# alexaiken/mpas-regent

Measured on AMD Instinct MI355X. Metric: Mcell-columns/sec per RK3 step; achieved HBM GB/s; x1.163842×56L, higher is better.
Workload: dtype f64; 1 GPU; x1.163842 x 56 levels, atm_srk3 (3 dyn_tend rk 0/1/2, 7 acoustic substeps); nCells=163842, nEdges=491520, nVertices=327680, nVertLevels=56, parallelism=single-gpu, exact=0, physics=0, transport=0, graph=1, fusedamp=1, fusesetup=1, smlsum=1, fusesml=1, defer4=1, ntu=1, mdamp=0

## Files before the change

mpas-regent_amd/csrc/k_acoustic.hip:

```cpp
#include "k_cols.h"
#include "mpas_dev.h"
#include "mpas_halo.h"

#include <type_traits>

namespace mpas {

template <int LP>
__device__ __forceinline__ double damp_edge(double rup, double d1, double d2, double t12, double spec, double coef,
                                            bool on) {
    return on ? rup + coef * (d2 - d1) * (1.0 - spec) / t12 : rup;
}

template <int LP, bool TME>
__device__ __forceinline__ void acoustic_orph_body(const DevState& S, double coefp, int ob) {
    const int L = S.L, k = (int)(threadIdx.x % LP);
    const int j = col_of<LP>(ob);
    if (j >= S.n_orph) return;
    const int e = fi(S, X_orph)[j];
    const int c1 = fi(S, F_cellsOnEdge)[(size_t)e * 2], c2 = fi(S, F_cellsOnEdge)[(size_t)e * 2 + 1];
    const double *dvi = fd(S, X_dvB), *tmf = fd(S, F_theta_m);
    const double ru = colk(fd(S, F_ru_p), e), d1 = colk(dvi, c1), d2 = colk(dvi, c2);
    const double t12 = TME ? colk(fd(S, X_tme), e) : colk(tmf, c1) + colk(tmf, c2);
    const int sh1 = fi(S, F_isShared)[c1], sh2 = fi(S, F_isShared)[c2];
    const bool on = (k < L) & !(sh1 & sh2);
    colk(fw(S, X_rupB), e) = PADW(damp_edge<LP>(ru, d1, d2, t12, fd(S, F_specZoneMaskEdge)[e], coefp, on));
}
template <int LP, bool TME>
__global__ __launch_bounds__(256) void k_acoustic_orph(DevState S, double coefp) {
    acoustic_orph_body<LP, TME>(S, coefp, (int)blockIdx.x);
}

template <int LP, bool EXACT, bool SELF, bool FIRST, bool MPASV, int MODE, bool TME, int SML, bool ACO = false,
          bool DD0 = false>
__device__ __forceinline__ void acoustic_body(const DevState& S, double dts, int small_step, double epssm, double resm,
                                              double coefp, int ncb, Blk bk, int wold = 1, int ddx = 0,
                                              double dtseps = 0.0) {
    static_assert(!(MPASV && MODE), "the deferred damping is the reference semantics' (physics 0)");
    static_assert(!(MPASV && ACO), "the MPAS forms load the stored set (recover changes theta_m)");
    static_assert(!(MPASV && DD0), "the MPAS forms' recover writes rw");
    static_assert(!(TME && ACO), "option tmedge keeps the stored set (its exact first launch would lose a wave)");
    static_assert(!SML || (FIRST && !MPASV), "set_smlstep precedes a stage's first substep (reference semantics)");
    static_assert(SML != 2 || !EXACT, "the flux sum reassociates: fast path only");
    const int L = S.L, k = (int)(threadIdx.x % LP);
    int blk = bk.b;
    blk = xcd_block_n(S.xcd, blk, ncb);
    const int c = col_of<LP>(blk) + S.lo[KC];
    if (c >= S.nCO) return;
    const size_t p = (size_t)c * LP + lpos(LP, k);
    double* rtp_f = fw(S, F_rtheta_pp);
    double* rpp_f = fw(S, F_rho_pp);
    double* rwp_f = fw(S, F_rw_p);
    double* ww_f = fw(S, F_wwAvg);
    const bool kl = k < L;
    const double spec = fd(S, F_specZoneMaskCell)[c];
    const int* eoc = fi(S, F_edgesOnCell) + (size_t)c * 10;
    const double* sgn = fd(S, F_edgesOnCellSign) + (size_t)c * 10;
    const int *cc1 = fi(S, X_ce_c1) + (size_t)c * 10, *cc2 = fi(S, X_ce_c2) + (size_t)c * 10;
    const double* cdv = fd(S, X_ce_dv) + (size_t)c * 10;
    const double invA = fd(S, F_invAreaCell)[c];
    const double *ru_p = fd(S, F_ru_p), *tm_f = fd(S, F_theta_m);
    const int *coth = fi(S, X_ce_oth) + (size_t)c * 10, *cs1 = fi(S, X_ce_s1) + (size_t)c * 10;
    int e_[NF], c1_[NF], c2_[NF], o_[NF], s1_[NF];
    double sgn_[NF], cdv_[NF], rup_[NF], t1_[NF], t2_[NF], ts_[NF];
    const int ne = SELF ? cell_rec<true>(S, c, e_, o_, s1_) : cell_rec<false>(S, c, e_, c1_, c2_);
    row_ld(sgn, sgn_);
    row_ld(cdv, cdv_);
    double rtp, rpp, rwp, ww, tm, tend_rho, w, coftz, zz, rz, cofwt, cofwz, cofwr, a_tri, alpha, rws, rw, dss;
    if constexpr (FIRST) {
        rtp = rpp = rwp = ww = 0.0;
    } else {
        col_rd2<LP>(rtp_f, rpp_f, c, k, L, rtp, rpp);
        col_rd2<LP>(rwp_f, ww_f, c, k, L, rwp, ww);
    }
    col_rd2<LP>(fd(S, F_theta_m), fd(S, F_tend_rho), c, k, L, tm, tend_rho);
    const uint8_t cpr = SML ? ((const uint8_t*)S.f[F_cprMask])[p] : 0;
    static_assert(NF % 2 == 0, "slot pairs");
#pragma unroll
    for (int i = 0; i < NF; i += 2) {
        gather2s<LP>(ru_p, e_[i], e_[i + 1], k, rup_[i], rup_[i + 1]);
        if constexpr (TME) {
            gather2s<LP>(fd(S, X_tme), e_[i], e_[i + 1], k, ts_[i], ts_[i + 1]);
        } else {
            cell_pair2<LP, SELF>(tm_f, c1_, c2_, o_, s1_, tm, i, k, t1_[i], t2_[i], t1_[i + 1], t2_[i + 1]);
            ts_[i] = t2_[i] + t1_[i];
            ts_[i + 1] = t2_[i + 1] + t1_[i + 1];
        }
    }
    int own = 0;
    if constexpr (MODE == 2) {
        const double* dvi = fd(S, X_dvB);
        const int* sh = fi(S, F_isShared);
        const double* spz = fd(S, F_specZoneMaskEdge);
        own = fi(S, X_eown)[c];
        const double dv_c = SELF ? colk(dvi, c) : 0.0;
        double d1_[NF], d2_[NF];
#pragma unroll
        for (int i = 0; i < NF; i += 2)
            cell_pair2<LP, SELF>(dvi, c1_, c2_, o_, s1_, dv_c, i, k, d1_[i], d2_[i], d1_[i + 1], d2_[i + 1]);
        int sh1_[NF], sh2_[NF];
        double spz_[NF];
#pragma unroll
        for (int i = 0; i < NF; i++) {
            const int x1 = SELF ? (s1_[i] ? c : o_[i]) : c1_[i], x2 = SELF ? (s1_[i] ? o_[i] : c) : c2_[i];
            sh1_[i] = sh[x1];
            sh2_[i] = sh[x2];
            spz_[i] = LP == 64 ? uniform_d(spz[e_[i]]) : spz[e_[i]];
        }
#pragma unroll
        for (int i = 0; i < NF; i++) {
            const bool on = kl & (e_[i] < S.nEdges) & !(sh1_[i] & sh2_[i]);
            rup_[i] = damp_edge<LP>(rup_[i], d1_[i], d2_[i], ts_[i], spz_[i], coefp, on);
        }
    }
    if constexpr (!ACO) col_rd2<LP>(fd(S, F_w), fd(S, F_coftz), c, k, L, w, coftz);
    else if constexpr (DD0) w = col_rd<LP>(fd(S, F_w), c, k, L);
    else if (ddx) col_rd2<LP>(fd(S, F_w), fd(S, F_dss), c, k, L, w, dss);
    else col_rd2<LP>(fd(S, F_w), fd(S, F_rw), c, k, L, w, rw);
    col_rd2<LP>(fd(S, F_zz), fd(S, F_rho_zz), c, k, L, zz, rz);
    const double fzm = fd(S, F_fzm)[k], fzp = fd(S, F_fzp)[k];
    int wst = 0;
    if constexpr (SML == 2) {
        double wn = w - colk(fd(S, X_smlS), c);
        wn *= (fzm * zz + fzp * lvl_dn<LP>(zz, k));
        const bool rz_ok = fi(S, F_bdyMaskCell)[c] <= kRelaxZone;
        wst = ((k <= L) & rz_ok & (cpr != 0)) ? 1 : ((k > L) & rz_ok) ? 2 : 0;
        if (wst == 1) w = wn;
    } else if constexpr (SML == 1) {
        const double* ut_f = fd(S, F_u_tend);
        const double *zb = fd(S, F_zb_cell), *zb3 = fd(S, F_zb3_cell);
        const double* sgnc = fd(S, F_edgesOnCell_sign) + (size_t)c * 10;
        double ut_[NF], utm_[NF], zb_[NF], zb3_[NF], sgs_[NF];
        row_ld(sgnc, sgs_);
#pragma unroll
        for (int i = 0; i < NF; i += 2) gather2s<LP>(ut_f, e_[i], e_[i + 1], k, ut_[i], ut_[i + 1]);
#pragma unroll
        for (int i = 0; i < NF; i++) {
            ut_[i] = ldz(k <= L, ut_[i]);
            gather2<LP>(zb, c * 10 + i, zb3, c * 10 + i, k, zb_[i], zb3_[i]);
        }
#pragma unroll
        for (int i = 0; i < NF; i++) utm_[i] = lvl_dn<LP>(ut_[i], k);
        double wn = w, sum = 0.0;
#pragma unroll
        for (int i = 0; i < NF; i++) {
            double flux = sgs_[i] * (fzm * ut_[i] + fzp * utm_[i]);
            const double t = (zb_[i] + copysign(1.0, ut_[i]) * zb3_[i]) * flux;
            if constexpr (EXACT) wn = sub_if(i < ne, wn, t);
            else sum = add_if(i < ne, sum, t);
        }
        for (int i = NF; i < ne; i++) {
            int iEdge = eoc[i];
            double ut = col_rd<LP>(ut_f, iEdge, k, L);
            double ut_m = lvl_dn<LP>(ut, k);
            double flux = sgnc[i] * (fzm * ut + fzp * ut_m);
            size_t q = ((size_t)c * 10 + i) * LP + lpos(LP, k);
            if constexpr (EXACT) wn -= (zb[q] + copysign(1.0, ut) * zb3[q]) * flux;
            else sum += (zb[q] + copysign(1.0, ut) * zb3[q]) * flux;
        }
        if constexpr (!EXACT) wn = w - sum;
        wn *= (fzm * zz + fzp * lvl_dn<LP>(zz, k));
        const bool rz_ok = fi(S, F_bdyMaskCell)[c] <= kRelaxZone;
        wst = ((k <= L) & rz_ok & (cpr != 0)) ? 1 : ((k > L) & rz_ok) ? 2 : 0;
        if (wst == 1) w = wn;
    }
    const double tw = (MPASV && S.physics == 2) ? col_rd<LP>(fd(S, F_tend_w), c, k, L) : w;
    col_rd2<LP>(fd(S, F_cofwt), fd(S, F_cofwz), c, k, L, cofwt, cofwz);
    if constexpr (!ACO) col_rd2<LP>(fd(S, F_cofwr), fd(S, F_a_tri), c, k, L, cofwr, a_tri);
    double dd;
    if constexpr (DD0) {
        col_rd2<LP>(fd(S, F_alpha_tri), fd(S, F_dss), c, k, L, alpha, dss);
        dd = 0.0;
    } else if (!MPASV && ddx) {
        col_rd2<LP>(fd(S, F_alpha_tri), fd(S, X_Dd), c, k, L, alpha, dd);
        if constexpr (!ACO) dss = col_rd<LP>(fd(S, F_dss), c, k, L);
    } else {
        col_rd2<LP>(fd(S, F_alpha_tri), fd(S, F_rw_save), c, k, L, alpha, rws);
        if constexpr (!ACO) col_rd2<LP>(fd(S, F_rw), fd(S, F_dss), c, k, L, rw, dss);
        else dss = col_rd<LP>(fd(S, F_dss), c, k, L);
        dd = rws - rw;
    }
    double gam = 0.0, tend_th = 0.0;
    if constexpr (MPASV) col_rd2<LP>(fd(S, F_gamma_tri), fd(S, F_tend_theta), c, k, L, gam, tend_th);
    const double tt = MPASV ? tend_th : tm;
    const double cofrz = fd(S, F_cofrz)[k], rdzw = fd(S, F_rdzw)[k];
    double coftz_L = 0.0;
    if constexpr (ACO) coftz_L = keepv<LP>(S, F_coftz, KC, c);
    if constexpr (MODE == 2) {
        double* rup_out = fw(S, X_rupB);
#pragma unroll
        for (int i = 0; i < NF; i++)
            if ((own >> i) & 1) colk(rup_out, e_[i]) = PADW(rup_[i]);
    }
    if constexpr (SML != 0) {
        if (wst == 1) {
            colk(fw(S, F_w), c) = w;
            if (k == L) keep_put<LP>(S, F_w, KC, c, w);
        } else if (wst == 2) {
            colk(fw(S, F_w), c) = 0.0;
        }
    }

    const double rtpo = (small_step == 0) ? 0 : rtp;
    const bool nst = MODE != 0 && (wold & 2);
    if (MODE == 0 || (wold & 1)) colk(fw(S, F_rtheta_pp_old), c) = KEEPW(rtpo, keepv<LP>(S, F_rtheta_pp_old, KC, c));
    auto store_div = [&](double rtp_new) {
        if constexpr (MODE != 0) colk(fw(S, X_dvA), c) = kl ? -(rtp_new - rtpo) : 0.0;
    };
    if (small_step == 0) {
        ww = 0;
        rwp = 0;
        if (kl) {
            rpp = 0;
            rtp = 0;
        }
    }

    auto damp_slot = [&](int i, double rpe) {
        const int e = eoc[i], x1 = cc1[i], x2 = cc2[i];
        const int sh1 = fi(S, F_isShared)[x1], sh2 = fi(S, F_isShared)[x2];
        const bool on = kl & (e < S.nEdges) & !(sh1 & sh2);
        rpe = damp_edge<LP>(rpe, colk(fd(S, X_dvB), x1), colk(fd(S, X_dvB), x2), colk(tm_f, x1) + colk(tm_f, x2),
                            fd(S, F_specZoneMaskEdge)[e], coefp, on);
        if ((own >> i) & 1) colk(fw(S, X_rupB), e) = PADW(rpe);
        return rpe;
    };

    if (spec != 0.0) {
        if constexpr (MODE == 2)
            for (int i = NF; i < ne; i++)
                if ((own >> i) & 1) damp_slot(i, colk(ru_p, eoc[i]));
        if (kl) {
            rpp = rpp + dts * tend_rho;
            rtp = rtp + dts * tt;
            rwp = rwp + dts * tw;
            ww = ww + 0.5 * (1.0 + epssm) * rwp;
        }
        if (!nst) {
            colk(rpp_f, c) = KEEPW(rpp, keepv<LP>(S, F_rho_pp, KC, c));
            colk(rtp_f, c) = KEEPW(rtp, keepv<LP>(S, F_rtheta_pp, KC, c));
            colk(rwp_f, c) = PADW(rwp);
            if (!(MPASV && (wold & 2))) colk(ww_f, c) = PADW(ww);
        }
        store_div(rtp);
        return;
    }

    double rs = 0, ts = 0;
#pragma unroll
    for (int i = 0; i < NF; i++) {
        double flux = sgn_[i] * dts * cdv_[i] * rup_[i] * invA;
        rs = sub_if(i < ne && kl, rs, flux);
        ts = sub_if(i < ne && kl, ts, flux * 0.5 * ts_[i]);
    }
    for (int i = NF; i < ne; i++) {
        double rpe = colk(ru_p, eoc[i]);
        if constexpr (MODE == 2) rpe = damp_slot(i, rpe);
        double flux = sgn[i] * dts * cdv[i] * ldz(kl, rpe) * invA;
        rs = sub_if(kl, rs, flux);
        ts = sub_if(kl, ts, flux * 0.5 * (ldz(kl, colk(tm_f, cc2[i])) + ldz(kl, colk(tm_f, cc1[i]))));
    }
    if constexpr (ACO) {
        const bool in = k >= 1 && k < L;
        const double zz_dn = lvl_dn<LP>(zz, k), tm_dn = lvl_dn<LP>(tm, k), rdzw_dn = lvl_dn<LP>(rdzw, k);
        cofwr = in ? vi_cofwr(dtseps, fzm, fzp, zz, zz_dn) : 0.0;
        coftz = in ? vi_coftz(dtseps, fzm, fzp, tm, tm_dn) : (k == L ? coftz_L : 0.0);
        a_tri = vi_a_tri(cofwz, lvl_dn<LP>(coftz, k), rdzw_dn, zz_dn, cofwr, dtseps * rdzw_dn, lvl_dn<LP>(cofwt, k));
    }
    const double rwp_p = lvl_up<LP>(rwp, k), coftz_p = lvl_up<LP>(coftz, k);
    rs = rpp + dts * tend_rho + rs - cofrz * resm * (rwp_p - rwp);
    ts = rtp + dts * tt + ts - resm * rdzw * (coftz_p * rwp_p - coftz * rwp);

    if constexpr (MPASV) {
        const double ts_m = lvl_dn<LP>(ts, k), rs_m = lvl_dn<LP>(rs, k);
        const double rtp_m = lvl_dn<LP>(rtp, k), rpp_m = lvl_dn<LP>(rpp, k);
// ... 90 lines not shown
        const double R0m = lvl_dn<LP>(R0, k), Rcm = lvl_dn<LP>(Rc, k);
        const double x0 = __shfl(rwold, (int)(threadIdx.x & 63) & ~(LP - 1), 64);
        double G = 1.0, H = 0.0;
        if (k >= 1 && k < L) {
            const double P = rwold + dts * w - cofwz * ((zz * ts) + resm * (zz * rtp)) - cofwr * (rs + resm * rpp) +
                             cofwt * (ts + resm * rtp);
            const double cT = cofwz * resm * zz_m + cofwt_m * resm;
            const double cR = cofwr * resm;
            const double F = 1.0 + dts * dss;
            const double Dd = dd;
            const double E = dts * dss * (fzm * zz + fzp * zz_m) * (fzm * rz + fzp * rz_m) * w;
            const double af = alpha / F;
            G = af * (cT * Tcm - cR * Rcm - a_tri);
            H = af * (P + cT * T0m - cR * R0m) + (Dd - E) / F - Dd;
            if (k == 1) {
                H = G * x0 + H;
                G = 0.0;
            }
        }
#pragma unroll
        for (int off = 1; off < LP; off <<= 1) {
            double Gp = __shfl_up(G, off, LP);
            double Hp = __shfl_up(H, off, LP);
            if (k >= off) {
                H = G * Hp + H;
                G = G * Gp;
            }
        }
        x = (k == 0) ? rwold : H;
    }
    if (k < L && k > 0) ww = ww + 0.5 * (1.0 - epssm) * rwold + 0.5 * (1.0 + epssm) * x;
    const double rtp_new = ts - rdzw * (coftz_p * rwp_p - coftz * x);
    if (!nst) {
        put2f<LP>(rpp_f, c, rtp_f, c, k, KEEPW(rs - cofrz * (rwp_p - x), keepv<LP>(S, F_rho_pp, KC, c)),
                 KEEPW(rtp_new, keepv<LP>(S, F_rtheta_pp, KC, c)));
        put2f<LP>(rwp_f, c, ww_f, c, k, PADW((k < L) ? x : rwp), PADW(ww));
    }
    store_div(rtp_new);
}
template <int LP, bool EXACT, bool SELF, bool FIRST, bool MPASV, int MODE, bool TME, int SML, bool ACO, bool DD0>
__global__ __launch_bounds__(256) void k_acoustic(DevState S, double dts, int small_step, double epssm, double resm,
                                                 double coefp, int ncb, int wold, int ddx, double dtseps) {
    acoustic_body<LP, EXACT, SELF, FIRST, MPASV, MODE, TME, SML, ACO, DD0>(S, dts, small_step, epssm, resm, coefp, ncb,
                                                                          this_blk(), wold, ddx, dtseps);
}
constexpr int kTailCells = 16384;
template <int LP, bool EXACT, bool SELF, bool FIRST, bool TME, int SML, bool ACO, bool DD0>
__global__ __launch_bounds__(256) void k_acoustic_o(DevState S, double dts, int small_step, double epssm, double resm,
                                                   double coefp, int ncb, int wold, int ddx, double dtseps) {
    const int b = (int)blockIdx.x;
    if (b < ncb)
        acoustic_body<LP, EXACT, SELF, FIRST, false, 2, TME, SML, ACO, DD0>(S, dts, small_step, epssm, resm, coefp,
                                                                             ncb, Blk{b, ncb}, wold, ddx, dtseps);
    else acoustic_orph_body<LP, TME>(S, coefp, b - ncb);
}
template <int LP, bool EXACT, bool SELF, int EPW, bool ACO, bool DD0>
__global__ __launch_bounds__(256) void k_hf_ac_vc(DevState S, double dts, int small_step, double epssm, double resm,
                                                 double coefp, int ncb, int nb1, int nVB, int wold, int ddx,
                                                 double dtseps) {
    const int b = (int)blockIdx.x;
    if (b < ncb)
        acoustic_body<LP, EXACT, SELF, false, false, 2, false, false, ACO, DD0>(S, dts, small_step, epssm, resm, coefp,
                                                                                 ncb, Blk{b, ncb}, wold, ddx, dtseps);
    else if (b < nb1) acoustic_orph_body<LP, false>(S, coefp, b - ncb);
    else solve_vc_body<LP, EPW, false>(S, nVB, 0, Blk{b - nb1, (int)gridDim.x - nb1});
}

template <int LP, int DD>
__global__ __launch_bounds__(256) void k_sml_flux(DevState S) {
    sml_flux_body<LP, DD>(S, this_blk());
}
template <int LP>
static hipError_t sml_flux_lp(const DevState& S, hipStream_t st, int dd) {
    if (dd < 0 || dd > 2) return hipErrorInvalidValue;
    auto run = [&](const DevState& X) {
        const int nb = col_blocks<LP>(X, KC);
        if (!nb) return;
// ... 132 lines not shown
                if (aco) go_td(ex, std::true_type{});
                else go_td(ex, std::false_type{});
            };
            if (exact) go_ta(std::true_type{});
            else go_ta(std::false_type{});
            return;
        }
        auto go = [&](auto ex, auto sf, auto md, auto ac, auto d0) {
            constexpr bool E = decltype(ex)::value, SF = decltype(sf)::value, A = decltype(ac)::value;
            constexpr bool D = decltype(d0)::value;
            constexpr int M = decltype(md)::value;
#define MPAS_AC(FI, MP, MM, TM, SM)                                                                                 \
    k_acoustic<LP, E, SF, FI, MP, MM, TM, SM, (A && !(MP) && !(TM)), (D && !(MP))><<<grid, 256, 0, st>>>( \
        X, dts, small_step, epssm, resm, coef_prev, ncb, wold, D ? 0 : ddx, dtseps)
            if constexpr (M == 0) {
                if (X.physics) {
                    if (first) MPAS_AC(true, true, 0, false, false);
                    else MPAS_AC(false, true, 0, false, false);
                    return;
                }
                if (tme) first ? MPAS_AC(true, false, 0, true, false) : MPAS_AC(false, false, 0, true, false);
                else first ? MPAS_AC(true, false, 0, false, false) : MPAS_AC(false, false, 0, false, false);
            } else {
                if (first) {
                    if constexpr (!E) {
                        if (sml == 2) {
                            tme ? MPAS_AC(true, false, M, true, 2) : MPAS_AC(true, false, M, false, 2);
                            return;
                        }
                    }
                    if (tme) sml ? MPAS_AC(true, false, M, true, 1) : MPAS_AC(true, false, M, true, 0);
                    else sml ? MPAS_AC(true, false, M, false, 1) : MPAS_AC(true, false, M, false, 0);
                } else {
                    if (tme) MPAS_AC(false, false, M, true, false);
                    else MPAS_AC(false, false, M, false, false);
                }
            }
#undef MPAS_AC
        };
        auto go_m = [&](auto ex, auto sf, auto ac, auto d0) {
            if (mode == 1) go(ex, sf, std::integral_constant<int, 1>{}, ac, d0);
            else if (mode == 2) go(ex, sf, std::integral_constant<int, 2>{}, ac, d0);
            else go(ex, sf, std::integral_constant<int, 0>{}, ac, d0);
        };
        auto go_s = [&](auto ex, auto ac, auto d0) {
            if (X.selfc) go_m(ex, std::true_type{}, ac, d0);
            else go_m(ex, std::false_type{}, ac, d0);
        };
        auto go_d = [&](auto ex, auto ac) {
            if (ddx == 2) go_s(ex, ac, std::true_type{});
            else go_s(ex, ac, std::false_type{});
        };
        auto go_a = [&](auto ex) {
            if (aco) go_d(ex, std::true_type{});
            else go_d(ex, std::false_type{});
        };
        if (exact) go_a(std::true_type{});
        else go_a(std::false_type{});
        if (mode == 2 && nob) {
            if (tme) k_acoustic_orph<LP, true><<<nob, 256, 0, st>>>(X, coef_prev);
            else k_acoustic_orph<LP, false><<<nob, 256, 0, st>>>(X, coef_prev);
        }
    };
    if (mode == 2 && sml == 1) HALO_RUN_R1(S, st, run, F_ru_p, F_ru_p, F_theta_m, X_dvB, F_u_tend);
    else if (mode == 2) HALO_RUN_R1(S, st, run, F_ru_p, F_ru_p, F_theta_m, X_dvB);
    else if (sml == 1) HALO_RUN_R1(S, st, run, F_ru_p, F_ru_p, F_theta_m, F_u_tend);
// ... 54 lines not shown
```

mpas-regent_amd/csrc/k_cols.h:

```cpp
#pragma once
#include "mpas_dev.h"

namespace mpas {

static inline int stream_grid_(size_t n) {
    size_t g = (n + 255) / 256;
    return (int)(g < 8192 ? (g ? g : 1) : 8192);
}

struct Pair64 {
    int pair, el;
    __host__ __device__ Pair64(int L) : pair(lpos(64, L) >> 1), el(lpos(64, L) & 1) {}
};
__device__ __forceinline__ void st64(double* d, size_t i, double2 v, Pair64 q) {
    if ((int)(i & 31) != q.pair) *(double2*)(d + 2 * i) = v;
    else d[2 * i + (1 - q.el)] = q.el ? v.x : v.y;
}
__device__ __forceinline__ void st64k(double* d, size_t i, double2 v, Pair64 q, double kl) {
    if ((int)(i & 31) == q.pair) {
        if (q.el) v.y = kl;
        else v.x = kl;
    }
    *(double2*)(d + 2 * i) = v;
}
// ... 452 lines not shown
#pragma unroll
    for (int i = 0; i < NF; i++) {
        double flux = sgs_[i] * (fzm * ut_[i] + fzp * utm_[i]);
        sum = add_if(i < ne, sum, (zb_[i] + copysign(1.0, ut_[i]) * zb3_[i]) * flux);
    }
    for (int i = NF; i < ne; i++) {
        int iEdge = eoc[i];
        double ut = col_rd<LP>(ut_f, iEdge, k, L);
        double ut_m = lvl_dn<LP>(ut, k);
        double flux = sgnc[i] * (fzm * ut + fzp * ut_m);
        size_t q = ((size_t)c * 10 + i) * LP + lpos(LP, k);
        sum += (zb[q] + copysign(1.0, ut) * zb3[q]) * flux;
    }
    colk(fw(S, X_smlS), c) = k <= L ? sum : 0.0;
    if constexpr (DD != 2) {
        double rws, rw;
        if constexpr (DD == 1) rws = rw = col_rd<LP>(fd(S, F_rw), c, k, L);
        else col_rd2<LP>(fd(S, F_rw_save), fd(S, F_rw), c, k, L, rws, rw);
        colk(fw(S, X_Dd), c) = k < L ? rws - rw : 0.0;
    }
}

template <int LP, bool MPASV = false, bool MD = false, int KEPT = 0, bool KD = false>
__device__ __forceinline__ void setup_vi_body(const DevState& S, int ncb, double dtseps, double rcv, double c2, Blk bk,
                                              int copies = 1) {
    static_assert(!KEPT || (!MPASV && !MD), "the kept setup: reference semantics");
    static_assert(!KD || KEPT, "kdiff from scratch: a kept launch");
    const int L = S.L, k = (int)(threadIdx.x % LP);
    int blk = bk.b;
    if constexpr (KEPT == 2) {
        const int c = col_of<LP>(xcd_block_n(S.xcd, blk, ncb)) + S.lo[KC];
        if (c >= S.nCO) return;
        double w, a, b, cc, alpha, gamma, gamma_old, kd = 0.0;
        gather2<LP>(fd(S, F_w), c, fd(S, X_a0), c, k, w, a);
        gather2<LP>(fd(S, X_b0), c, fd(S, X_c0), c, k, b, cc);
        if constexpr (KD) gather2<LP>(fd(S, F_gamma_tri), c, fd(S, X_kd0), c, k, gamma_old, kd);
        else gamma_old = colk(fd(S, F_gamma_tri), c);
        vi_alpha_gamma<LP>(a, b, cc, gamma_old, k, alpha, gamma);
        put2f<LP>(fw(S, F_w_2), c, fw(S, F_alpha_tri), c, k, KEEPW(w, keepv<LP>(S, F_w_2, KC, c)),
                  vi_alpha_st<LP>(S, c, k, alpha));
        if constexpr (KD)
            put2f<LP>(fw(S, F_gamma_tri), c, fw(S, F_kdiff), c, k, vi_gamma_st<LP>(S, c, k, gamma),
                      KEEPW(kd, keepv<LP>(S, F_kdiff, KC, c)));
        else colk(fw(S, F_gamma_tri), c) = vi_gamma_st<LP>(S, c, k, gamma);
        if (c == 0 && k < L) fw(S, F_cofrz)[k] = dtseps * fd(S, F_rdzw)[k];
        return;
    } else if constexpr (KEPT == 1) {
        const int c = col_of<LP>(xcd_block_n(S.xcd, blk, ncb)) + S.lo[KC];
        if (c >= S.nCO) return;
        if constexpr (KD) colk(fw(S, F_kdiff), c) = KEEPW(colk(fd(S, X_kd0), c), keepv<LP>(S, F_kdiff, KC, c));
        double rtp, w, tm, zz, exner, rb, rtb, exb;
        gather2<LP>(fd(S, F_rtheta_p), c, fd(S, F_w), c, k, rtp, w);
        gather2<LP>(fd(S, F_theta_m), c, fd(S, F_zz), c, k, tm, zz);
        gather2<LP>(fd(S, F_exner), c, fd(S, F_rho_base), c, k, exner, rb);
        gather2<LP>(fd(S, F_rtheta_base), c, fd(S, F_exner_base), c, k, rtb, exb);
        const double gamma_old = colk(fd(S, F_gamma_tri), c);
        const double coftz_old = k == L ? keepv<LP>(S, F_coftz, KC, c) : 0.0;
        colk(fw(S, F_w_2), c) = KEEPW(w, keepv<LP>(S, F_w_2, KC, c));
        const double q_k = 0.0, q_km1 = 0.0, qtotal = 0.5 * (q_k + q_km1);
        const double cqw = k > L ? 0.0 : 1.0 / (1.0 + qtotal), qtot = 0.0;
        vi_column<LP, false>(S, c, k, zz, exner, tm, cqw, qtot, rb, rtb, rtp, exb, gamma_old, coftz_old, dtseps, rcv, c2,
                             true, (copies & 2) != 0, (copies & 4) != 0);
        return;
    }
    if (blk >= ncb) {
        const int e = col_of<LP>(xcd_block_n(S.xcd, blk - ncb, bk.n - ncb)) + S.lo[KE];
        if (e >= S.nEO) return;
        if (copies & 1) {
            double ru, u;
            gather2<LP>(fd(S, F_ru), e, fd(S, F_u), e, k, ru, u);
// ... 42 lines not shown
```

mpas-regent_amd/csrc/mpas_dev.h:

```cpp
#pragma once
#include <hip/hip_runtime.h>
#include <stdint.h>

namespace mpas {

__host__ __device__ constexpr int lpos(int LP, int k) { return LP == 64 ? (((k & 31) << 1) | (k >> 5)) : k; }
__host__ __device__ constexpr int plev(int LP, int p) { return LP == 64 ? ((p >> 1) | ((p & 1) << 5)) : p; }

constexpr int kPairW = 8;
__host__ __device__ constexpr size_t vidx(int W, int LP, size_t e, int i, int k) {
    return W == kPairW ? ((e * (kPairW / 2) + (size_t)(i >> 1)) * LP + (size_t)k) * 2 + (size_t)(i & 1)
                       : (e * W + (size_t)i) * LP + (size_t)lpos(LP, k);
}

enum FieldKind { K_C3, K_C3V, K_E3, K_V3, K_C2F, K_C2I, K_E2F, K_E2I, K_V2F, K_V2I, K_C3B, K_ZV };
enum FieldDist { D_U = 0, D_Z = 1, D_B = 2, D_M = 3, D_S = 4 };

enum FieldId {
#define MPAS_FIELD(name, KIND, W, DIST, LO, HI) F_##name,
#include "mpas_fields.def"
#undef MPAS_FIELD
    F_COUNT,
    X_cosAngleEdge = F_COUNT,
    X_cosLatEdge,
// ... 383 lines not shown
static void* bounds_symbol_() {
    void* p = nullptr;
    return hipGetSymbolAddress(&p, HIP_SYMBOL(g_bounds)) == hipSuccess ? p : nullptr;
}
static const int g_bounds_registered_ = bounds_register_tu(&bounds_symbol_);
__device__ __noinline__ static inline void* bounds_chk(const void* base, const void* p, unsigned bytes) {
    BoundsTab* t = g_bounds;
    if (!t) return (void*)p;
    const unsigned long long b = (unsigned long long)base, a = (unsigned long long)p;
    int lo = 0, hi = t->n - 1, hit = -1;
    while (lo <= hi) {
        const int mid = (lo + hi) >> 1;
        if (t->lo[mid] <= b) hit = mid, lo = mid + 1;
        else hi = mid - 1;
    }
    if (hit < 0 || b >= t->hi[hit]) return (void*)p;
    if (a >= t->lo[hit] && a + bytes <= t->hi[hit]) return (void*)p;
    if (atomicAdd(&t->count, 1u) == 0u) {
        t->addr = a;
        t->field_lo = t->lo[hit];
        t->where = ((unsigned long long)blockIdx.x << 32) | threadIdx.x;
    }
    return g_bounds_sink;
}
#define MPAS_CHK(base, p, bytes) bounds_chk((base), (p), (bytes))
#else
#define MPAS_CHK(base, p, bytes) (p)
#endif

template <int LP>
__device__ __forceinline__ uint32_t col_off(int ent, int k) {
    return ((uint32_t)ent * (uint32_t)LP + (uint32_t)lpos(LP, k)) * (uint32_t)sizeof(double);
}
template <class T>
__device__ __forceinline__ T& at_off(T* f, uint32_t off) {
#if MPAS_BOUNDS
    return *(T*)bounds_chk(f, (const char*)f + off, sizeof(T));
#else
    return *(T*)((MPAS_GLOBAL char*)(f) + off);
#endif
}
#define colk(f, ent) at_off((f), col_off<LP>((ent), k))


__device__ __forceinline__ void swap_halves(double& x, double& y) {
    int2 xi = __builtin_bit_cast(int2, x), yi = __builtin_bit_cast(int2, y);
    const auto r0 = __builtin_amdgcn_permlane32_swap(xi.x, yi.x, false, false);
    const auto r1 = __builtin_amdgcn_permlane32_swap(xi.y, yi.y, false, false);
    xi.x = (int)r0[0];
    yi.x = (int)r0[1];
    xi.y = (int)r1[0];
    yi.y = (int)r1[1];
    x = __builtin_bit_cast(double, xi);
    y = __builtin_bit_cast(double, yi);
}
template <int LP>
__device__ __forceinline__ void gather2(const double* fa, int ia, const double* fb, int ib, int k, double& a,
                                        double& b) {
    if constexpr (LP == 64) {
        const bool hi = k >= 32;
        const char* base = hi ? (const char*)fb + (size_t)(uint32_t)ib * 512 : (const char*)fa + (size_t)(uint32_t)ia * 512;
        const double2 t = *(const double2*)MPAS_CHK(hi ? fb : fa, base + (k & 31) * 16, 16);
        double x = t.x, y = t.y;
        swap_halves(x, y);
        a = x;
        b = y;
    } else {
        a = colk(fa, ia);
        b = colk(fb, ib);
    }
}

template <int LP>
__device__ __forceinline__ double2 gather2_ld(const double* fa, int ia, const double* fb, int ib, int k) {
    if constexpr (LP == 64) {
        const bool hi = k >= 32;
        const char* base = hi ? (const char*)fb + (size_t)(uint32_t)ib * 512 : (const char*)fa + (size_t)(uint32_t)ia * 512;
        return *(const double2*)MPAS_CHK(hi ? fb : fa, base + (k & 31) * 16, 16);
    } else {
        return make_double2(colk(fa, ia), colk(fb, ib));
    }
}
template <int LP>
__device__ __forceinline__ double2 gather2s_ld(const double* f, int ia, int ib, int k) {
    if constexpr (LP == 64) {
        const uint32_t off = (uint32_t)(k >= 32 ? ib : ia) * 512u + (uint32_t)(k & 31) * 16u;
        return at_off((const double2*)f, off);
    } else {
        return make_double2(colk(f, ia), colk(f, ib));
    }
}
template <int LP>
__device__ __forceinline__ void g2_fin(double2 t, double& a, double& b) {
    double x = t.x, y = t.y;
    if constexpr (LP == 64) swap_halves(x, y);
    a = x;
    b = y;
}

template <int LP, bool SELF>
__device__ __forceinline__ void cell_pair(const double* f, int c1, int c2, int oth, int s1, double own, int k,
                                          double& x1, double& x2) {
    if constexpr (SELF) {
        const double xo = colk(f, oth);
        x1 = s1 ? own : xo;
        x2 = s1 ? xo : own;
    } else {
        x1 = colk(f, c1);
        x2 = colk(f, c2);
    }
}

template <int LP>
__device__ __forceinline__ void put2(double* fa, int ia, double* fb, int ib, int k, double a, double b, bool oka,
                                     bool okb) {
    if constexpr (LP == 64) {
        double x = a, y = b;
        swap_halves(x, y);
        const auto f = __builtin_amdgcn_permlane32_swap((unsigned)oka, (unsigned)okb, false, false);
        const bool sx = f[0] != 0, sy = f[1] != 0;
        const bool hi = k >= 32;
        char* base = hi ? (char*)fb + (size_t)(uint32_t)ib * 512 : (char*)fa + (size_t)(uint32_t)ia * 512;
        double* q = (double*)MPAS_CHK(hi ? fb : fa, base + (k & 31) * 16, 16);
        if (sx && sy) *(double2*)q = make_double2(x, y);
        else if (sx) q[0] = x;
        else if (sy) q[1] = y;
    } else {
        if (oka) colk(fa, ia) = a;
        if (okb) colk(fb, ib) = b;
    }
}

template <int LP>
__device__ __forceinline__ void put2f(double* fa, int ia, double* fb, int ib, int k, double a, double b) {
    if constexpr (LP == 64) {
        double x = a, y = b;
        swap_halves(x, y);
        const bool hi = k >= 32;
        char* base = hi ? (char*)fb + (size_t)(uint32_t)ib * 512 : (char*)fa + (size_t)(uint32_t)ia * 512;
        *(double2*)MPAS_CHK(hi ? fb : fa, base + (k & 31) * 16, 16) = make_double2(x, y);
    } else {
        colk(fa, ia) = a;
        colk(fb, ib) = b;
    }
}

template <int LP>
__device__ __forceinline__ void gather2s(const double* f, int ia, int ib, int k, double& a, double& b) {
    if constexpr (LP == 64) {
        const uint32_t off = (uint32_t)(k >= 32 ? ib : ia) * 512u + (uint32_t)(k & 31) * 16u;
        const double2 t = at_off((const double2*)f, off);
        double x = t.x, y = t.y;
        swap_halves(x, y);
        a = x;
        b = y;
    } else {
        a = colk(f, ia);
        b = colk(f, ib);
    }
}

template <int LP, bool SELF>
__device__ __forceinline__ void cell_pair2(const double* f, const int* c1, const int* c2, const int* oth, const int* s1,
                                           double own, int i, int k, double& x1, double& x2, double& y1, double& y2) {
    if constexpr (SELF) {
        double xo, yo;
        gather2s<LP>(f, oth[i], oth[i + 1], k, xo, yo);
        x1 = s1[i] ? own : xo;
        x2 = s1[i] ? xo : own;
        y1 = s1[i + 1] ? own : yo;
        y2 = s1[i + 1] ? yo : own;
    } else {
        gather2s<LP>(f, c1[i], c2[i], k, x1, x2);
        gather2s<LP>(f, c1[i + 1], c2[i + 1], k, y1, y2);
    }
}
// ... 45 lines not shown
    int r[CREC];
    row_ld(fi(S, SELF ? X_cRs : X_cR) + (size_t)c * CREC, r);
#pragma unroll
    for (int i = 0; i < NF; i++) {
        e_[i] = r[i];
        a_[i] = r[NF + i];
        b_[i] = r[2 * NF + i];
    }
    return r[3 * NF];
}

#define PADW(v) (k > L ? 0.0 : (v))

template <int LP>
__device__ __forceinline__ const double* keep_tail(const DevState& S, int f, int kind, bool lev0) {
    const int n = kind == KC ? S.nCells : kind == KE ? S.nEdges : S.nVertices;
    return fd(S, f) + (size_t)(n + 1) * LP + (lev0 ? (size_t)(n + 1) : 0);
}
template <int LP>
__device__ __forceinline__ double keepv(const DevState& S, int f, int kind, int ent, bool lev0 = false) {
    return ldc(keep_tail<LP>(S, f, kind, lev0) + ent);
}
template <int LP>
__device__ __forceinline__ void keep_put(const DevState& S, int f, int kind, int ent, double v) {
    const_cast<double*>(keep_tail<LP>(S, f, kind, false))[ent] = v;
}
template <int LP>
__device__ __forceinline__ void keep_put0(const DevState& S, int f, int kind, int ent, double v) {
    const_cast<double*>(keep_tail<LP>(S, f, kind, true))[ent] = v;
}
#define KEEPW(v, kl_) (k == L ? (kl_) : PADW(v))
#define KEEPW0(v, k0_, kl_) (k == 0 ? (k0_) : KEEPW(v, kl_))

template <int LP>
__device__ __forceinline__ double col_rd(const double* f, int ent, int k, int L) {
    return ldz(k <= L, at_off(f, col_off<LP>(ent, k)));
}
template <int LP>
__device__ __forceinline__ void col_rd2(const double* f, const double* g, int ent, int k, int L, double& a, double& b) {
    gather2<LP>(f, ent, g, ent, k, a, b);
    a = ldz(k <= L, a);
    b = ldz(k <= L, b);
}
#endif

}

#define MPAS_LP_DISPATCH(LPVAL, FN, ...)                              \
    do {                                                              \
        switch (LPVAL) {                                              \
            case 8: return FN<8>(__VA_ARGS__);                        \
            case 16: return FN<16>(__VA_ARGS__);                      \
            case 32: return FN<32>(__VA_ARGS__);                      \
            case 64: return FN<64>(__VA_ARGS__);                      \
            default: return hipErrorInvalidValue;                     \
        }                                                             \
    } while (0)
```

Measured before the change: 49.39 Mcell-columns/s.

## Use nontemporal loads/stores for streaming acoustic fields and add no-store substep variant

Adds nontemporal load/store helpers selected by a compile-time MPAS_NT bitmask, and applies them to single-use column reads and writes in the acoustic kernel and the vertical-implicit setup. This aims to keep streaming data from evicting reused edge gathers from cache. It also adds an NST specialization for the default no-store substep that skips reading wwAvg, and dispatches to it when wold&2. Nontemporal hints can backfire if the data is actually reused by the next kernel through L2/MALL.

```diff
diff --git a/mpas-regent_amd/csrc/k_acoustic.hip b/mpas-regent_amd/csrc/k_acoustic.hip
--- a/mpas-regent_amd/csrc/k_acoustic.hip
+++ b/mpas-regent_amd/csrc/k_acoustic.hip
@@ -32,7 +32,7 @@
 }
 
 template <int LP, bool EXACT, bool SELF, bool FIRST, bool MPASV, int MODE, bool TME, int SML, bool ACO = false,
-          bool DD0 = false>
+          bool DD0 = false, bool NST = false>
 __device__ __forceinline__ void acoustic_body(const DevState& S, double dts, int small_step, double epssm, double resm,
                                               double coefp, int ncb, Blk bk, int wold = 1, int ddx = 0,
                                               double dtseps = 0.0) {
@@ -42,6 +42,7 @@
     static_assert(!(TME && ACO), "option tmedge keeps the stored set (its exact first launch would lose a wave)");
     static_assert(!SML || (FIRST && !MPASV), "set_smlstep precedes a stage's first substep (reference semantics)");
     static_assert(SML != 2 || !EXACT, "the flux sum reassociates: fast path only");
+    static_assert(!NST || (!EXACT && !FIRST && MODE == 2 && !TME && ACO && DD0), "the default step's -st launch");
     const int L = S.L, k = (int)(threadIdx.x % LP);
     int blk = bk.b;
     blk = xcd_block_n(S.xcd, blk, ncb);
@@ -53,6 +54,7 @@
     double* rwp_f = fw(S, F_rw_p);
     double* ww_f = fw(S, F_wwAvg);
     const bool kl = k < L;
+    constexpr bool N1 = nt_group(1), N2 = nt_group(2), N3 = nt_group(4);
     const double spec = fd(S, F_specZoneMaskCell)[c];
     const int* eoc = fi(S, F_edgesOnCell) + (size_t)c * 10;
     const double* sgn = fd(S, F_edgesOnCellSign) + (size_t)c * 10;
@@ -70,11 +72,12 @@
     if constexpr (FIRST) {
         rtp = rpp = rwp = ww = 0.0;
     } else {
-        col_rd2<LP>(rtp_f, rpp_f, c, k, L, rtp, rpp);
-        col_rd2<LP>(rwp_f, ww_f, c, k, L, rwp, ww);
+        col_rd2<LP, N2>(rtp_f, rpp_f, c, k, L, rtp, rpp);
+        if constexpr (NST) rwp = col_rd<LP, N2>(rwp_f, c, k, L), ww = 0.0;
+        else col_rd2<LP, N2>(rwp_f, ww_f, c, k, L, rwp, ww);
     }
     col_rd2<LP>(fd(S, F_theta_m), fd(S, F_tend_rho), c, k, L, tm, tend_rho);
-    const uint8_t cpr = SML ? ((const uint8_t*)S.f[F_cprMask])[p] : 0;
+    const uint8_t cpr = SML ? ld_off<N1>((const uint8_t*)S.f[F_cprMask], (uint32_t)p) : 0;
     static_assert(NF % 2 == 0, "slot pairs");
 #pragma unroll
     for (int i = 0; i < NF; i += 2) {
@@ -113,15 +116,15 @@
             rup_[i] = damp_edge<LP>(rup_[i], d1_[i], d2_[i], ts_[i], spz_[i], coefp, on);
         }
     }
-    if constexpr (!ACO) col_rd2<LP>(fd(S, F_w), fd(S, F_coftz), c, k, L, w, coftz);
-    else if constexpr (DD0) w = col_rd<LP>(fd(S, F_w), c, k, L);
-    else if (ddx) col_rd2<LP>(fd(S, F_w), fd(S, F_dss), c, k, L, w, dss);
-    else col_rd2<LP>(fd(S, F_w), fd(S, F_rw), c, k, L, w, rw);
-    col_rd2<LP>(fd(S, F_zz), fd(S, F_rho_zz), c, k, L, zz, rz);
+    if constexpr (!ACO) col_rd2<LP, N1>(fd(S, F_w), fd(S, F_coftz), c, k, L, w, coftz);
+    else if constexpr (DD0) w = col_rd<LP, N1>(fd(S, F_w), c, k, L);
+    else if (ddx) col_rd2<LP, N1>(fd(S, F_w), fd(S, F_dss), c, k, L, w, dss);
+    else col_rd2<LP, N1>(fd(S, F_w), fd(S, F_rw), c, k, L, w, rw);
+    col_rd2<LP, N1>(fd(S, F_zz), fd(S, F_rho_zz), c, k, L, zz, rz);
     const double fzm = fd(S, F_fzm)[k], fzp = fd(S, F_fzp)[k];
     int wst = 0;
     if constexpr (SML == 2) {
-        double wn = w - colk(fd(S, X_smlS), c);
+        double wn = w - colk_ld(N1, fd(S, X_smlS), c);
         wn *= (fzm * zz + fzp * lvl_dn<LP>(zz, k));
         const bool rz_ok = fi(S, F_bdyMaskCell)[c] <= kRelaxZone;
         wst = ((k <= L) & rz_ok & (cpr != 0)) ? 1 : ((k > L) & rz_ok) ? 2 : 0;
@@ -165,19 +168,19 @@
         if (wst == 1) w = wn;
     }
     const double tw = (MPASV && S.physics == 2) ? col_rd<LP>(fd(S, F_tend_w), c, k, L) : w;
-    col_rd2<LP>(fd(S, F_cofwt), fd(S, F_cofwz), c, k, L, cofwt, cofwz);
-    if constexpr (!ACO) col_rd2<LP>(fd(S, F_cofwr), fd(S, F_a_tri), c, k, L, cofwr, a_tri);
+    col_rd2<LP, N1>(fd(S, F_cofwt), fd(S, F_cofwz), c, k, L, cofwt, cofwz);
+    if constexpr (!ACO) col_rd2<LP, N1>(fd(S, F_cofwr), fd(S, F_a_tri), c, k, L, cofwr, a_tri);
     double dd;
     if constexpr (DD0) {
-        col_rd2<LP>(fd(S, F_alpha_tri), fd(S, F_dss), c, k, L, alpha, dss);
+        col_rd2<LP, N1>(fd(S, F_alpha_tri), fd(S, F_dss), c, k, L, alpha, dss);
         dd = 0.0;
     } else if (!MPASV && ddx) {
-        col_rd2<LP>(fd(S, F_alpha_tri), fd(S, X_Dd), c, k, L, alpha, dd);
-        if constexpr (!ACO) dss = col_rd<LP>(fd(S, F_dss), c, k, L);
+        col_rd2<LP, N1>(fd(S, F_alpha_tri), fd(S, X_Dd), c, k, L, alpha, dd);
+        if constexpr (!ACO) dss = col_rd<LP, N1>(fd(S, F_dss), c, k, L);
     } else {
-        col_rd2<LP>(fd(S, F_alpha_tri), fd(S, F_rw_save), c, k, L, alpha, rws);
-        if constexpr (!ACO) col_rd2<LP>(fd(S, F_rw), fd(S, F_dss), c, k, L, rw, dss);
-        else dss = col_rd<LP>(fd(S, F_dss), c, k, L);
+        col_rd2<LP, N1>(fd(S, F_alpha_tri), fd(S, F_rw_save), c, k, L, alpha, rws);
+        if constexpr (!ACO) col_rd2<LP, N1>(fd(S, F_rw), fd(S, F_dss), c, k, L, rw, dss);
+        else dss = col_rd<LP, N1>(fd(S, F_dss), c, k, L);
         dd = rws - rw;
     }
     double gam = 0.0, tend_th = 0.0;
@@ -190,7 +193,7 @@
         double* rup_out = fw(S, X_rupB);
 #pragma unroll
         for (int i = 0; i < NF; i++)
-            if ((own >> i) & 1) colk(rup_out, e_[i]) = PADW(rup_[i]);
+            if ((own >> i) & 1) colk_st(N3, rup_out, e_[i], PADW(rup_[i]));
     }
     if constexpr (SML != 0) {
         if (wst == 1) {
@@ -202,10 +205,10 @@
     }
 
     const double rtpo = (small_step == 0) ? 0 : rtp;
-    const bool nst = MODE != 0 && (wold & 2);
+    const bool nst = NST || (MODE != 0 && (wold & 2));
     if (MODE == 0 || (wold & 1)) colk(fw(S, F_rtheta_pp_old), c) = KEEPW(rtpo, keepv<LP>(S, F_rtheta_pp_old, KC, c));
     auto store_div = [&](double rtp_new) {
-        if constexpr (MODE != 0) colk(fw(S, X_dvA), c) = kl ? -(rtp_new - rtpo) : 0.0;
+        if constexpr (MODE != 0) colk_st(N3, fw(S, X_dvA), c, kl ? -(rtp_new - rtpo) : 0.0);
     };
     if (small_step == 0) {
         ww = 0;
@@ -222,7 +225,7 @@
         const bool on = kl & (e < S.nEdges) & !(sh1 & sh2);
         rpe = damp_edge<LP>(rpe, colk(fd(S, X_dvB), x1), colk(fd(S, X_dvB), x2), colk(tm_f, x1) + colk(tm_f, x2),
                             fd(S, F_specZoneMaskEdge)[e], coefp, on);
-        if ((own >> i) & 1) colk(fw(S, X_rupB), e) = PADW(rpe);
+        if ((own >> i) & 1) colk_st(N3, fw(S, X_rupB), e, PADW(rpe));
         return rpe;
     };
 
@@ -237,10 +240,10 @@
             ww = ww + 0.5 * (1.0 + epssm) * rwp;
         }
         if (!nst) {
-            colk(rpp_f, c) = KEEPW(rpp, keepv<LP>(S, F_rho_pp, KC, c));
-            colk(rtp_f, c) = KEEPW(rtp, keepv<LP>(S, F_rtheta_pp, KC, c));
-            colk(rwp_f, c) = PADW(rwp);
-            if (!(MPASV && (wold & 2))) colk(ww_f, c) = PADW(ww);
+            colk_st(N3, rpp_f, c, KEEPW(rpp, keepv<LP>(S, F_rho_pp, KC, c)));
+            colk_st(N3, rtp_f, c, KEEPW(rtp, keepv<LP>(S, F_rtheta_pp, KC, c)));
+            colk_st(N3, rwp_f, c, PADW(rwp));
+            if (!(MPASV && (wold & 2))) colk_st(N3, ww_f, c, PADW(ww));
         }
         store_div(rtp);
         return;
@@ -397,17 +400,18 @@
     if (k < L && k > 0) ww = ww + 0.5 * (1.0 - epssm) * rwold + 0.5 * (1.0 + epssm) * x;
     const double rtp_new = ts - rdzw * (coftz_p * rwp_p - coftz * x);
     if (!nst) {
-        put2f<LP>(rpp_f, c, rtp_f, c, k, KEEPW(rs - cofrz * (rwp_p - x), keepv<LP>(S, F_rho_pp, KC, c)),
-                 KEEPW(rtp_new, keepv<LP>(S, F_rtheta_pp, KC, c)));
-        put2f<LP>(rwp_f, c, ww_f, c, k, PADW((k < L) ? x : rwp), PADW(ww));
+        put2f<LP, N3>(rpp_f, c, rtp_f, c, k, KEEPW(rs - cofrz * (rwp_p - x), keepv<LP>(S, F_rho_pp, KC, c)),
+                     KEEPW(rtp_new, keepv<LP>(S, F_rtheta_pp, KC, c)));
+        put2f<LP, N3>(rwp_f, c, ww_f, c, k, PADW((k < L) ? x : rwp), PADW(ww));
     }
     store_div(rtp_new);
 }
-template <int LP, bool EXACT, bool SELF, bool FIRST, bool MPASV, int MODE, bool TME, int SML, bool ACO, bool DD0>
+template <int LP, bool EXACT, bool SELF, bool FIRST, bool MPASV, int MODE, bool TME, int SML, bool ACO, bool DD0,
+          bool NST = false>
 __global__ __launch_bounds__(256) void k_acoustic(DevState S, double dts, int small_step, double epssm, double resm,
                                                  double coefp, int ncb, int wold, int ddx, double dtseps) {
-    acoustic_body<LP, EXACT, SELF, FIRST, MPASV, MODE, TME, SML, ACO, DD0>(S, dts, small_step, epssm, resm, coefp, ncb,
-                                                                          this_blk(), wold, ddx, dtseps);
+    acoustic_body<LP, EXACT, SELF, FIRST, MPASV, MODE, TME, SML, ACO, DD0, NST>(S, dts, small_step, epssm, resm, coefp,
+                                                                               ncb, this_blk(), wold, ddx, dtseps);
 }
 constexpr int kTailCells = 16384;
 template <int LP, bool EXACT, bool SELF, bool FIRST, bool TME, int SML, bool ACO, bool DD0>
@@ -606,6 +610,13 @@
                     if (tme) sml ? MPAS_AC(true, false, M, true, 1) : MPAS_AC(true, false, M, true, 0);
                     else sml ? MPAS_AC(true, false, M, false, 1) : MPAS_AC(true, false, M, false, 0);
                 } else {
+                    if constexpr (M == 2 && !E && A && D) {
+                        if (!tme && (wold & 2)) {
+                            k_acoustic<LP, false, SF, false, false, 2, false, 0, true, true, true>
+                                <<<grid, 256, 0, st>>>(X, dts, small_step, epssm, resm, coef_prev, ncb, wold, 0, dtseps);
+                            return;
+                        }
+                    }
                     if (tme) MPAS_AC(false, false, M, true, false);
                     else MPAS_AC(false, false, M, false, false);
                 }
diff --git a/mpas-regent_amd/csrc/k_cols.h b/mpas-regent_amd/csrc/k_cols.h
--- a/mpas-regent_amd/csrc/k_cols.h
+++ b/mpas-regent_amd/csrc/k_cols.h
@@ -508,10 +508,11 @@
         const int c = col_of<LP>(xcd_block_n(S.xcd, blk, ncb)) + S.lo[KC];
         if (c >= S.nCO) return;
         double w, a, b, cc, alpha, gamma, gamma_old, kd = 0.0;
-        gather2<LP>(fd(S, F_w), c, fd(S, X_a0), c, k, w, a);
-        gather2<LP>(fd(S, X_b0), c, fd(S, X_c0), c, k, b, cc);
-        if constexpr (KD) gather2<LP>(fd(S, F_gamma_tri), c, fd(S, X_kd0), c, k, gamma_old, kd);
-        else gamma_old = colk(fd(S, F_gamma_tri), c);
+        constexpr bool NT = nt_group(8);
+        gather2<LP, NT>(fd(S, F_w), c, fd(S, X_a0), c, k, w, a);
+        gather2<LP, NT>(fd(S, X_b0), c, fd(S, X_c0), c, k, b, cc);
+        if constexpr (KD) gather2<LP, NT>(fd(S, F_gamma_tri), c, fd(S, X_kd0), c, k, gamma_old, kd);
+        else gamma_old = colk_ld(NT, fd(S, F_gamma_tri), c);
         vi_alpha_gamma<LP>(a, b, cc, gamma_old, k, alpha, gamma);
         put2f<LP>(fw(S, F_w_2), c, fw(S, F_alpha_tri), c, k, KEEPW(w, keepv<LP>(S, F_w_2, KC, c)),
                   vi_alpha_st<LP>(S, c, k, alpha));
diff --git a/mpas-regent_amd/csrc/mpas_dev.h b/mpas-regent_amd/csrc/mpas_dev.h
--- a/mpas-regent_amd/csrc/mpas_dev.h
+++ b/mpas-regent_amd/csrc/mpas_dev.h
@@ -439,6 +439,37 @@
 __device__ __forceinline__ uint32_t col_off(int ent, int k) {
     return ((uint32_t)ent * (uint32_t)LP + (uint32_t)lpos(LP, k)) * (uint32_t)sizeof(double);
 }
+#ifndef MPAS_NT
+#define MPAS_NT 14
+#endif
+constexpr bool nt_group(int bit) { return (MPAS_NT & bit) != 0; }
+typedef double d2v __attribute__((ext_vector_type(2)));
+__device__ __forceinline__ double2 ld2_nt(const void* p) {
+    const d2v t = __builtin_nontemporal_load((const d2v*)p);
+    return make_double2(t.x, t.y);
+}
+__device__ __forceinline__ void st2_nt(void* p, double x, double y) {
+    d2v t;
+    t.x = x;
+    t.y = y;
+    __builtin_nontemporal_store(t, (d2v*)p);
+}
+template <class T>
+__device__ __forceinline__ T ld_off_nt(const T* f, uint32_t off) {
+#if MPAS_BOUNDS
+    return __builtin_nontemporal_load((const T*)bounds_chk(f, (const char*)f + off, sizeof(T)));
+#else
+    return __builtin_nontemporal_load((const MPAS_GLOBAL T*)((const MPAS_GLOBAL char*)(f) + off));
+#endif
+}
+template <class T>
+__device__ __forceinline__ void st_off_nt(T* f, uint32_t off, T v) {
+#if MPAS_BOUNDS
+    __builtin_nontemporal_store(v, (T*)bounds_chk(f, (const char*)f + off, sizeof(T)));
+#else
+    __builtin_nontemporal_store(v, (MPAS_GLOBAL T*)((MPAS_GLOBAL char*)(f) + off));
+#endif
+}
 template <class T>
 __device__ __forceinline__ T& at_off(T* f, uint32_t off) {
 #if MPAS_BOUNDS
@@ -448,6 +479,18 @@
 #endif
 }
 #define colk(f, ent) at_off((f), col_off<LP>((ent), k))
+template <bool NT, class T>
+__device__ __forceinline__ T ld_off(const T* f, uint32_t off) {
+    if constexpr (NT) return ld_off_nt(f, off);
+    else return at_off(f, off);
+}
+template <bool NT, class T>
+__device__ __forceinline__ void st_off(T* f, uint32_t off, T v) {
+    if constexpr (NT) st_off_nt(f, off, v);
+    else at_off(f, off) = v;
+}
+#define colk_ld(NT, f, ent) ld_off<(NT)>((f), col_off<LP>((ent), k))
+#define colk_st(NT, f, ent, v) st_off<(NT)>((f), col_off<LP>((ent), k), (v))
 
 
 __device__ __forceinline__ void swap_halves(double& x, double& y) {
@@ -461,20 +504,22 @@
     x = __builtin_bit_cast(double, xi);
     y = __builtin_bit_cast(double, yi);
 }
-template <int LP>
+template <int LP, bool NT = false>
 __device__ __forceinline__ void gather2(const double* fa, int ia, const double* fb, int ib, int k, double& a,
                                         double& b) {
     if constexpr (LP == 64) {
         const bool hi = k >= 32;
         const char* base = hi ? (const char*)fb + (size_t)(uint32_t)ib * 512 : (const char*)fa + (size_t)(uint32_t)ia * 512;
-        const double2 t = *(const double2*)MPAS_CHK(hi ? fb : fa, base + (k & 31) * 16, 16);
+        double2 t;
+        if constexpr (NT) t = ld2_nt(MPAS_CHK(hi ? fb : fa, base + (k & 31) * 16, 16));
+        else t = *(const double2*)MPAS_CHK(hi ? fb : fa, base + (k & 31) * 16, 16);
         double x = t.x, y = t.y;
         swap_halves(x, y);
         a = x;
         b = y;
     } else {
-        a = colk(fa, ia);
-        b = colk(fb, ib);
+        a = colk_ld(NT, fa, ia);
+        b = colk_ld(NT, fb, ib);
     }
 }
 
@@ -538,17 +583,18 @@
     }
 }
 
-template <int LP>
+template <int LP, bool NT = false>
 __device__ __forceinline__ void put2f(double* fa, int ia, double* fb, int ib, int k, double a, double b) {
     if constexpr (LP == 64) {
         double x = a, y = b;
         swap_halves(x, y);
         const bool hi = k >= 32;
         char* base = hi ? (char*)fb + (size_t)(uint32_t)ib * 512 : (char*)fa + (size_t)(uint32_t)ia * 512;
-        *(double2*)MPAS_CHK(hi ? fb : fa, base + (k & 31) * 16, 16) = make_double2(x, y);
-    } else {
-        colk(fa, ia) = a;
-        colk(fb, ib) = b;
+        if constexpr (NT) st2_nt(MPAS_CHK(hi ? fb : fa, base + (k & 31) * 16, 16), x, y);
+        else *(double2*)MPAS_CHK(hi ? fb : fa, base + (k & 31) * 16, 16) = make_double2(x, y);
+    } else {
+        colk_st(NT, fa, ia, a);
+        colk_st(NT, fb, ib, b);
     }
 }
 
@@ -660,13 +706,13 @@
 #define KEEPW(v, kl_) (k == L ? (kl_) : PADW(v))
 #define KEEPW0(v, k0_, kl_) (k == 0 ? (k0_) : KEEPW(v, kl_))
 
-template <int LP>
+template <int LP, bool NT = false>
 __device__ __forceinline__ double col_rd(const double* f, int ent, int k, int L) {
-    return ldz(k <= L, at_off(f, col_off<LP>(ent, k)));
-}
-template <int LP>
+    return ldz(k <= L, ld_off<NT>(f, col_off<LP>(ent, k)));
+}
+template <int LP, bool NT = false>
 __device__ __forceinline__ void col_rd2(const double* f, const double* g, int ent, int k, int L, double& a, double& b) {
-    gather2<LP>(f, ent, g, ent, k, a, b);
+    gather2<LP, NT>(f, ent, g, ent, k, a, b);
     a = ldz(k <= L, a);
     b = ldz(k <= L, b);
 }
```

After: 51.27 Mcell-columns/s (median of 6 runs). 3.8% higher.
